# caishiqing/voice-tts

Measured on AMD Instinct MI355X. Metric: audio_seconds_per_second, higher is better.
Workload: dtype bf16

## Files before the change

### voice-tts_amd/csrc/gemm_x6.hip

```cpp
#include "common.h"

namespace ixtts {

typedef float gx_f32x16 __attribute__((ext_vector_type(16)));
typedef __bf16 gx_bf16x8 __attribute__((ext_vector_type(8)));
typedef float gx_f32x4 __attribute__((ext_vector_type(4)));
typedef unsigned int gx_u32x4 __attribute__((ext_vector_type(4)));


__global__ void gemm_x6_pack_kernel(const float* __restrict__ w, uint4* __restrict__ out, int N, int K, int Npad) {
  const long total = (long)(K / 8) * Npad;
  for (long idx = blockIdx.x * (long)blockDim.x + threadIdx.x; idx < total; idx += (long)gridDim.x * blockDim.x) {
    const int n = (int)(idx % Npad);
    const int ko = (int)(idx / Npad);
    float v[8];
#pragma unroll
    for (int e = 0; e < 8; ++e) v[e] = n < N ? w[(long)n * K + ko * 8 + e] : 0.f;
    uint4 ph, pm, pl;
    split8_bf16x3(v, ph, pm, pl);
    const int g = ko >> 1, kh = ko & 1;
    uint4* base = out + ((long)g * 6) * Npad + n;
    base[(long)(0 * 2 + kh) * Npad] = ph;
    base[(long)(1 * 2 + kh) * Npad] = pm;
    base[(long)(2 * 2 + kh) * Npad] = pl;
  }
}

__global__ __launch_bounds__(256) void gemm_x6_split_kernel(const float* __restrict__ a, long lda, uint4* __restrict__ out, int M, int K, long Mpad) {
  __shared__ float tile[64][65];
  const int r0 = blockIdx.x * 64, k0 = blockIdx.y * 64;
  const int t = threadIdx.x;
#pragma unroll
  for (int i = 0; i < 4; ++i) {
    const int r = (t >> 4) + 16 * i, kq = t & 15;
    float4 v = make_float4(0.f, 0.f, 0.f, 0.f);
    if (r0 + r < M) v = *reinterpret_cast<const float4*>(a + (long)(r0 + r) * lda + k0 + 4 * kq);
    tile[r][4 * kq + 0] = v.x; tile[r][4 * kq + 1] = v.y; tile[r][4 * kq + 2] = v.z; tile[r][4 * kq + 3] = v.w;
  }
  __syncthreads();
#pragma unroll
  for (int u = 0; u < 2; ++u) {
    const int r = t & 63, o = (t >> 6) + 4 * u;
    float v[8];
#pragma unroll
    for (int e = 0; e < 8; ++e) v[e] = tile[r][o * 8 + e];
    uint4 ph, pm, pl;
    split8_bf16x3(v, ph, pm, pl);
    const int ko = (k0 >> 3) + o, g = ko >> 1, kh = ko & 1;
    uint4* base = out + ((long)g * 6) * Mpad + r0 + r;
    base[(long)(0 * 2 + kh) * Mpad] = ph;
    base[(long)(1 * 2 + kh) * Mpad] = pm;
    base[(long)(2 * 2 + kh) * Mpad] = pl;
  }
}

enum { EPI_PLAIN = 0, EPI_SWIGLU = 1, EPI_GATE = 2 };

struct GemmX6Params {
  const uint4* Ap;
  long Mpad;
  long arow0;
  const uint4* Wp;
  const float* bias;
  float* C;
  long ldc;
  int M, N, Npad, K, accumulate, m_tiles, n_tiles;
  int tap_steps;
  int epi;
  const float* gate;
  long gate_ld, rows_per_batch;
  int nbatch;
  const int* gate_seq_off;
  unsigned long long* dbg;
};


template <int MT, int NT, int NST, int DBG = 0>
__global__ __launch_bounds__(256, (NST * (MT + NT) * 6 * 64 * 16 <= 80 * 1024) ? 2 : 1) void gemm_x6_kernel(GemmX6Params p) {
  constexpr int BM = 64 * MT, BN = 64 * NT;
  constexpr int A_UNITS = 6 * BM, W_UNITS = 6 * BN, STAGE = A_UNITS + W_UNITS;
  constexpr int NDMA = (6 * (MT + NT)) / 4;
  static_assert((6 * (MT + NT)) % 4 == 0, "the copies are dealt evenly to the 4 waves");
  constexpr int D = NST - 1;
  extern __shared__ uint4 smem[];

  const int nwg = p.m_tiles * p.n_tiles;
  const int bid = blockIdx.x;
  const int xcd = bid & 7, idx = bid >> 3;
  const int qd = nwg >> 3, rm = nwg & 7;
  const int lin = (xcd < rm ? xcd * (qd + 1) : rm * (qd + 1) + (xcd - rm) * qd) + idx;
  const int m_tile = lin / p.n_tiles, n_tile = lin - m_tile * p.n_tiles;
  const int m0 = m_tile * BM, n0 = n_tile * BN;

  const int tid = threadIdx.x, lane = tid & 63, wave = tid >> 6;
  const int wm = wave >> 1, wn = wave & 1;
  const int l31 = lane & 31, lh = lane >> 5;

  gx_f32x16 acc[MT][NT];
#pragma unroll
  for (int i = 0; i < MT; ++i)
#pragma unroll
    for (int j = 0; j < NT; ++j)
#pragma unroll
      for (int r = 0; r < 16; ++r) acc[i][j][r] = 0.f;

  const uint4* asrc = p.Ap + p.arow0 + m0 + lane;
  const uint4* wsrc = p.Wp + n0 + lane;
  auto issue = [&](int s, uint4* st) {
    const int tap = s / p.tap_steps, sa = s - tap * p.tap_steps;
#pragma unroll
    for (int q = 0; q < NDMA; ++q) {
      const int e = q * 4 + wave;
      if (e < 6 * MT) {
        const int run = e / MT, piece = e % MT;
        __builtin_amdgcn_global_load_lds((const __attribute__((address_space(1))) void*)(asrc + ((long)sa * 6 + run) * p.Mpad + tap + piece * 64),
                                         (__attribute__((address_space(3))) void*)(st + run * BM + piece * 64), 16, 0, 0);
      } else {
        const int e2 = e - 6 * MT, run = e2 / NT, piece = e2 % NT;
        __builtin_amdgcn_global_load_lds((const __attribute__((address_space(1))) void*)(wsrc + ((long)s * 6 + run) * p.Npad + piece * 64),
                                         (__attribute__((address_space(3))) void*)(st + A_UNITS + run * BN + piece * 64), 16, 0, 0);
      }
    }
  };

  const int steps = p.K >> 4;
  auto wg_stamp = [&](int k) {
    if constexpr (DBG == 3) {
      if (tid == 0) p.dbg[128 + (long)blockIdx.x * 4 + k] = __builtin_amdgcn_s_memrealtime();
    }
  };
  auto wait_younger = [&](int y) {
    if (y >= 2) asm volatile("s_waitcnt vmcnt(%0)" ::"n"(2 * NDMA) : "memory");
    else if (y == 1) asm volatile("s_waitcnt vmcnt(%0)" ::"n"(NDMA) : "memory");
    else asm volatile("s_waitcnt vmcnt(0)" ::: "memory");
  };
  static_assert(D >= 1 && D <= 3, "1..3 steps of copies in flight behind the one waited for");
  wg_stamp(0);
  for (int t = 0; t < D && t < steps; ++t) issue(t, smem + t * STAGE);
  wait_younger(min(D, steps) - 1);
  __builtin_amdgcn_s_barrier();
  asm volatile("" ::: "memory");
  wg_stamp(1);

  const unsigned base_addr = (unsigned)(uintptr_t)(const __attribute__((address_space(3))) void*)smem;
  int st_cur = 0, st_nxt = D % NST;
  for (int s = 0; s < steps; ++s) {
    auto stamp = [&](int k) {
      if constexpr (DBG == 3) {
        if (blockIdx.x == 0 && tid == 0 && s < 16) {
          p.dbg[s * 8 + k] = __builtin_amdgcn_s_memtime();
          if (k == 0) p.dbg[s * 8 + 7] = __builtin_amdgcn_s_memrealtime();
        }
      }
    };
    stamp(0);
    if (DBG != 1 && s + D < steps) issue(s + D, smem + st_nxt * STAGE);
    stamp(1);
    const unsigned cur_addr = base_addr + (unsigned)(st_cur * STAGE * 16);
    if constexpr (DBG != 2) {
      gx_u32x4 af[3][MT], bf[3][NT];
      const unsigned aaddr = cur_addr + (unsigned)((lh * BM + wm * (32 * MT) + l31) * 16);
      const unsigned waddr = cur_addr + (unsigned)((A_UNITS + lh * BN + wn * (32 * NT) + l31) * 16);
      if constexpr (MT == 4 && NT == 2) {
        asm volatile(
            "ds_read_b128 %0, %18 offset:%20\n ds_read_b128 %1, %18 offset:%21\n ds_read_b128 %2, %18 offset:%22\n ds_read_b128 %3, %18 offset:%23\n"
            "ds_read_b128 %4, %18 offset:%24\n ds_read_b128 %5, %18 offset:%25\n ds_read_b128 %6, %18 offset:%26\n ds_read_b128 %7, %18 offset:%27\n"
            "ds_read_b128 %8, %18 offset:%28\n ds_read_b128 %9, %18 offset:%29\n ds_read_b128 %10, %18 offset:%30\n ds_read_b128 %11, %18 offset:%31\n"
            "ds_read_b128 %12, %19 offset:%32\n ds_read_b128 %13, %19 offset:%33\n ds_read_b128 %14, %19 offset:%34\n ds_read_b128 %15, %19 offset:%35\n"
            "ds_read_b128 %16, %19 offset:%36\n ds_read_b128 %17, %19 offset:%37\n s_waitcnt lgkmcnt(0)"
            : "=&v"(af[0][0]), "=&v"(af[0][1]), "=&v"(af[0][2]), "=&v"(af[0][3]), "=&v"(af[1][0]), "=&v"(af[1][1]), "=&v"(af[1][2]), "=&v"(af[1][3]),
              "=&v"(af[2][0]), "=&v"(af[2][1]), "=&v"(af[2][2]), "=&v"(af[2][3]), "=&v"(bf[0][0]), "=&v"(bf[0][1]), "=&v"(bf[1][0]), "=&v"(bf[1][1]),
              "=&v"(bf[2][0]), "=&v"(bf[2][1])
            : "v"(aaddr), "v"(waddr), "n"((0 * 2 * BM + 0) * 16), "n"((0 * 2 * BM + 32) * 16), "n"((0 * 2 * BM + 64) * 16), "n"((0 * 2 * BM + 96) * 16),
              "n"((1 * 2 * BM + 0) * 16), "n"((1 * 2 * BM + 32) * 16), "n"((1 * 2 * BM + 64) * 16), "n"((1 * 2 * BM + 96) * 16), "n"((2 * 2 * BM + 0) * 16),
              "n"((2 * 2 * BM + 32) * 16), "n"((2 * 2 * BM + 64) * 16), "n"((2 * 2 * BM + 96) * 16), "n"((0 * 2 * BN + 0) * 16), "n"((0 * 2 * BN + 32) * 16),
              "n"((1 * 2 * BN + 0) * 16), "n"((1 * 2 * BN + 32) * 16), "n"((2 * 2 * BN + 0) * 16), "n"((2 * 2 * BN + 32) * 16)
            : "memory");
      } else {
        static_assert(MT == 2 && NT == 2, "fragment block written for 256 x 128 and 128 x 128 tiles");
        asm volatile(
            "ds_read_b128 %0, %12 offset:%14\n ds_read_b128 %1, %12 offset:%15\n ds_read_b128 %2, %12 offset:%16\n ds_read_b128 %3, %12 offset:%17\n"
            "ds_read_b128 %4, %12 offset:%18\n ds_read_b128 %5, %12 offset:%19\n ds_read_b128 %6, %13 offset:%20\n ds_read_b128 %7, %13 offset:%21\n"
            "ds_read_b128 %8, %13 offset:%22\n ds_read_b128 %9, %13 offset:%23\n ds_read_b128 %10, %13 offset:%24\n ds_read_b128 %11, %13 offset:%25\n"
            "s_waitcnt lgkmcnt(0)"
            : "=&v"(af[0][0]), "=&v"(af[0][1]), "=&v"(af[1][0]), "=&v"(af[1][1]), "=&v"(af[2][0]), "=&v"(af[2][1]), "=&v"(bf[0][0]), "=&v"(bf[0][1]),
              "=&v"(bf[1][0]), "=&v"(bf[1][1]), "=&v"(bf[2][0]), "=&v"(bf[2][1])
            : "v"(aaddr), "v"(waddr), "n"((0 * 2 * BM + 0) * 16), "n"((0 * 2 * BM + 32) * 16), "n"((1 * 2 * BM + 0) * 16), "n"((1 * 2 * BM + 32) * 16),
              "n"((2 * 2 * BM + 0) * 16), "n"((2 * 2 * BM + 32) * 16), "n"((0 * 2 * BN + 0) * 16), "n"((0 * 2 * BN + 32) * 16), "n"((1 * 2 * BN + 0) * 16),
              "n"((1 * 2 * BN + 32) * 16), "n"((2 * 2 * BN + 0) * 16), "n"((2 * 2 * BN + 32) * 16)
            : "memory");
      }
      stamp(2);
#pragma unroll
      for (int i = 0; i < MT; ++i)
#pragma unroll
        for (int j = 0; j < NT; ++j) {
          const gx_bf16x8 ah = __builtin_bit_cast(gx_bf16x8, af[0][i]), am = __builtin_bit_cast(gx_bf16x8, af[1][i]), al = __builtin_bit_cast(gx_bf16x8, af[2][i]);
          const gx_bf16x8 bh = __builtin_bit_cast(gx_bf16x8, bf[0][j]), bm = __builtin_bit_cast(gx_bf16x8, bf[1][j]), bl = __builtin_bit_cast(gx_bf16x8, bf[2][j]);
          acc[i][j] = __builtin_amdgcn_mfma_f32_32x32x16_bf16(al, bh, acc[i][j], 0, 0, 0);
          acc[i][j] = __builtin_amdgcn_mfma_f32_32x32x16_bf16(ah, bl, acc[i][j], 0, 0, 0);
          acc[i][j] = __builtin_amdgcn_mfma_f32_32x32x16_bf16(am, bm, acc[i][j], 0, 0, 0);
          acc[i][j] = __builtin_amdgcn_mfma_f32_32x32x16_bf16(am, bh, acc[i][j], 0, 0, 0);
          acc[i][j] = __builtin_amdgcn_mfma_f32_32x32x16_bf16(ah, bm, acc[i][j], 0, 0, 0);
          acc[i][j] = __builtin_amdgcn_mfma_f32_32x32x16_bf16(ah, bh, acc[i][j], 0, 0, 0);
        }
      if constexpr (DBG == 3) asm volatile("" ::"v"(acc[0][0][0]), "v"(acc[MT - 1][NT - 1][15]));
    }
    stamp(3);
    wait_younger(DBG == 1 ? 0 : max(0, min(D - 1, steps - s - 2)));
    stamp(4);
    __builtin_amdgcn_s_barrier();
    asm volatile("" ::: "memory");
    stamp(5);
    st_cur = st_cur + 1 == NST ? 0 : st_cur + 1;
    st_nxt = st_nxt + 1 == NST ? 0 : st_nxt + 1;
  }

  wg_stamp(2);
  if (p.epi != EPI_PLAIN) {
    static_assert(NT == 2, "pair epilogues: the wave's two 32-column blocks are the two halves");
    const int oc = (n0 + wn * 64) / 2 + l31;
    const int nh = p.N >> 1;
    if (oc < nh) {
      const float ba = p.bias != nullptr ? p.bias[n0 + wn * 64 + l31] : 0.f, bb = p.bias != nullptr ? p.bias[n0 + wn * 64 + 32 + l31] : 0.f;
#pragma unroll
      for (int i = 0; i < MT; ++i) {
        const int rbase = m0 + wm * (32 * MT) + i * 32 + 4 * lh;
#pragma unroll
        for (int r = 0; r < 16; ++r) {
          const int row = rbase + (r & 3) + 8 * (r >> 2);
          if (row < p.M) {
            float a = acc[i][0][r] + ba, b = acc[i][1][r] + bb, v;
            if (p.epi == EPI_SWIGLU) {
              v = a / (1.0f + expf(-a)) * b;
            } else {
              const long gb = p.gate_seq_off ? (long)seq_of_row(p.gate_seq_off, p.nbatch, row) : min((long)row / p.rows_per_batch, (long)p.nbatch - 1);
              const float* g = p.gate + gb * p.gate_ld;
              a += g[oc];
              b += g[nh + oc];
              v = tanhf(a) * (1.0f / (1.0f + expf(-b)));
            }
            p.C[(long)row * p.ldc + oc] = v;
          }
        }
      }
    }
  } else
#pragma unroll
  for (int j = 0; j < NT; ++j) {
    const int col = n0 + wn * (32 * NT) + j * 32 + l31;
    const bool col_ok = col < p.N;
    const float bv = (p.bias != nullptr && col_ok) ? p.bias[col] : 0.f;
#pragma unroll
    for (int i = 0; i < MT; ++i) {
      const int rbase = m0 + wm * (32 * MT) + i * 32 + 4 * lh;
#pragma unroll
      for (int r = 0; r < 16; ++r) {
        const int row = rbase + (r & 3) + 8 * (r >> 2);
        if (col_ok && row < p.M) {
          float* c = p.C + (long)row * p.ldc + col;
          float v = acc[i][j][r] + bv;
          if (p.accumulate) v += *c;
          *c = v;
        }
      }
    }
  }
  if constexpr (DBG == 3) {
    asm volatile("s_waitcnt vmcnt(0)" ::: "memory");
    wg_stamp(3);
  }
}

template <int MT, int NT, int NST, int DBG = 0>
static int launch_gemm_x6(GemmX6Params p, hipStream_t st) {
  constexpr int BM = 64 * MT, BN = 64 * NT;
  constexpr size_t smem = (size_t)NST * (6 * BM + 6 * BN) * 16;
  static_assert(smem <= 160 * 1024, "LDS stages of this tile shape");
  p.m_tiles = ceil_div(p.M, BM);
  p.n_tiles = ceil_div(p.N, BN);
  IX_ARG((long)p.n_tiles * BN <= p.Npad, "gemm_x6: packed weights padded to %d features, the %d-wide tile needs %d", p.Npad, BN, p.n_tiles * BN);
  const int taps = (p.K >> 4) / p.tap_steps;
  IX_ARG(p.arow0 + (long)p.m_tiles * BM + taps - 1 <= p.Mpad, "gemm_x6: activation planes hold %ld rows, the %d-row tiles reach row %ld", p.Mpad, BM,
         p.arow0 + (long)p.m_tiles * BM + taps - 1);
  auto kern = gemm_x6_kernel<MT, NT, NST, DBG>;
  static bool done = false;
  if (!done) {
    IX_HIP(hipFuncSetAttribute((const void*)kern, hipFuncAttributeMaxDynamicSharedMemorySize, (int)smem));
    done = true;
  }
  hipLaunchKernelGGL(kern, dim3(p.m_tiles * p.n_tiles), dim3(256), smem, st, p);
  IX_HIP(hipGetLastError());
  return IXTTS_OK;
}

}

using namespace ixtts;

extern "C" size_t ixtts_gemm_x6_packed_bytes(int N, int K) {
  if (N <= 0 || K <= 0 || K % 64) return 0;
  const size_t Npad = (size_t)(N + 255) / 256 * 256;
  return (size_t)(K / 16) * 6 * Npad * 16;
}

extern "C" int ixtts_gemm_x6_pack(const float* w_dev, void* packed_dev, int N, int K, void* stream) {
  IX_ARG(w_dev && packed_dev && N > 0 && K > 0 && K % 64 == 0, "gemm_x6_pack: bad argument (K must be a multiple of 64)");
  const int Npad = (N + 255) / 256 * 256;
  const long total = (long)(K / 8) * Npad;
  hipLaunchKernelGGL(gemm_x6_pack_kernel, dim3((unsigned)std::min<long>((total + 255) / 256, 4096)), dim3(256), 0, (hipStream_t)stream, w_dev,
                     reinterpret_cast<uint4*>(packed_dev), N, K, Npad);
  IX_HIP(hipGetLastError());
  return IXTTS_OK;
}

extern "C" long ixtts_gemm_x6_rows_padded(long rows) { return rows <= 0 ? 0 : (rows + 255) / 256 * 256 + 256; }

extern "C" int ixtts_gemm_x6_split(const float* a_dev, long lda, void* planes_dev, long rows, int K, void* stream) {
  IX_ARG(a_dev && planes_dev && rows > 0 && K > 0 && K % 64 == 0, "gemm_x6_split: bad argument (K must be a multiple of 64)");
  IX_ARG(lda >= K && lda % 4 == 0 && (reinterpret_cast<uintptr_t>(a_dev) & 15) == 0, "gemm_x6_split: rows must be 16-byte aligned (lda %ld)", lda);
  const long Mpad = ixtts_gemm_x6_rows_padded(rows);
  hipLaunchKernelGGL(gemm_x6_split_kernel, dim3((unsigned)(Mpad / 64), K / 64), dim3(256), 0, (hipStream_t)stream, a_dev, lda,
                     reinterpret_cast<uint4*>(planes_dev), (int)rows, K, Mpad);
  IX_HIP(hipGetLastError());
  return IXTTS_OK;
}

static int run_gemm_x6(GemmX6Params p, int tile, hipStream_t st) {
  if (tile == 0) {
    const long t42 = (long)ceil_div(p.M, 256) * ceil_div(p.N, 128);
    tile = t42 >= 140 ? 2 : 3;
  }
  switch (tile) {
    case 2: return launch_gemm_x6<4, 2, 2>(p, st);
    case 3: return launch_gemm_x6<2, 2, 3>(p, st);
    case 4: return launch_gemm_x6<4, 2, 4>(p, st);
    case 5: return launch_gemm_x6<2, 2, 4>(p, st);
    case 12: return launch_gemm_x6<4, 2, 2, 1>(p, st);
    case 22: return launch_gemm_x6<4, 2, 2, 2>(p, st);
    case 32: return launch_gemm_x6<4, 2, 2, 3>(p, st);
    case 33: return launch_gemm_x6<2, 2, 3, 3>(p, st);
  }
  set_error("gemm_x6: tile %d (0 auto; 2 / 3: 256x128 / 128x128, two workgroups per CU; 4 / 5: the same, one per CU with a 4-stage ring)", tile);
  return IXTTS_ERR_ARG;
}

extern "C" int ixtts_gemm_x6_f32(const void* a_planes_dev, long rows_total, long row0, const void* packed_dev, const float* bias_dev, float* c_dev,
                                 long ldc, int M, int N, int K, int accumulate, int tile, void* stream) {
  IX_ARG(a_planes_dev && packed_dev && c_dev && M > 0 && N > 0 && K > 0 && K % 64 == 0, "gemm_x6: bad argument (K must be a multiple of 64: the split pass works on 64-wide k blocks)");
  IX_ARG(ldc >= N && row0 >= 0 && row0 + M <= rows_total, "gemm_x6: rows [%ld, %ld) of %ld, ldc %ld", row0, row0 + M, rows_total, ldc);
  GemmX6Params p;
  p.Ap = reinterpret_cast<const uint4*>(a_planes_dev); p.Mpad = ixtts_gemm_x6_rows_padded(rows_total); p.arow0 = row0;
  p.Wp = reinterpret_cast<const uint4*>(packed_dev); p.bias = bias_dev; p.C = c_dev; p.ldc = ldc;
  p.M = M; p.N = N; p.Npad = (N + 255) / 256 * 256; p.K = K; p.accumulate = accumulate ? 1 : 0; p.m_tiles = p.n_tiles = 0;
  p.tap_steps = K >> 4; p.epi = EPI_PLAIN; p.gate = nullptr; p.gate_ld = 0; p.rows_per_batch = 1; p.nbatch = 1; p.gate_seq_off = nullptr;
  p.dbg = (tile == 32 || tile == 33) ? reinterpret_cast<unsigned long long*>(const_cast<float*>(bias_dev)) : nullptr;
  if (p.dbg) p.bias = nullptr;
  return run_gemm_x6(p, tile, (hipStream_t)stream);
}

extern "C" int ixtts_gemm_x6_pair_f32(const void* a_planes_dev, long rows_total, long row0, int taps, const void* packed_dev, const float* bias_dev,
                                      const float* gate_dev, long gate_ld, long rows_per_batch, int nbatch, float* c_dev, long ldc, int M, int N, int K,
                                      int epilogue, int tile, void* stream) {
  IX_ARG(a_planes_dev && packed_dev && c_dev && M > 0 && N > 0 && taps > 0 && K > 0, "gemm_x6_pair: bad argument");
  IX_ARG(K % taps == 0 && (K / taps) % 64 == 0 && N % 64 == 0, "gemm_x6_pair: K %d = %d taps of a multiple of 64, N %d a multiple of 64", K, taps, N);
  IX_ARG(epilogue == EPI_SWIGLU || (epilogue == EPI_GATE && gate_dev && rows_per_batch > 0 && nbatch > 0 && gate_ld >= N / 2),
         "gemm_x6_pair: epilogue %d (1 swiglu; 2 gate, with gate biases)", epilogue);
  IX_ARG(ldc >= N / 2 && row0 >= 0 && row0 + M + taps - 1 <= rows_total, "gemm_x6_pair: rows [%ld, %ld) + %d taps of %ld, ldc %ld", row0, row0 + M, taps,
         rows_total, ldc);
  IX_ARG(tile == 0 || tile == 2 || tile == 3, "gemm_x6_pair: tile %d (0 auto, 2, 3)", tile);
  GemmX6Params p;
  p.Ap = reinterpret_cast<const uint4*>(a_planes_dev); p.Mpad = ixtts_gemm_x6_rows_padded(rows_total); p.arow0 = row0;
  p.Wp = reinterpret_cast<const uint4*>(packed_dev); p.bias = bias_dev; p.C = c_dev; p.ldc = ldc;
  p.M = M; p.N = N; p.Npad = (N + 255) / 256 * 256; p.K = K; p.accumulate = 0; p.m_tiles = p.n_tiles = 0;
  p.tap_steps = (K / taps) >> 4; p.epi = epilogue; p.gate = gate_dev; p.gate_ld = gate_ld; p.rows_per_batch = rows_per_batch; p.nbatch = nbatch;
  p.gate_seq_off = nullptr;
  p.dbg = nullptr;
  return run_gemm_x6(p, tile, (hipStream_t)stream);
}

extern "C" int ixtts_gemm_x6_pair_gate_varlen_f32(const void* a_planes_dev, long rows_total, long row0, int taps, const void* packed_dev, const float* bias_dev,
                                                  const float* gate_dev, long gate_ld, const int* seq_off_dev, int nseq, float* c_dev, long ldc, int M, int N,
                                                  int K, int tile, void* stream) {
  IX_ARG(seq_off_dev && nseq > 0, "gemm_x6_pair_gate_varlen: null offsets table or nseq %d", nseq);
  IX_ARG(a_planes_dev && packed_dev && c_dev && gate_dev && M > 0 && N > 0 && taps > 0 && K > 0 && gate_ld >= N / 2, "gemm_x6_pair_gate_varlen: bad argument");
  IX_ARG(K % taps == 0 && (K / taps) % 64 == 0 && N % 64 == 0, "gemm_x6_pair_gate_varlen: K %d = %d taps of a multiple of 64, N %d a multiple of 64", K, taps, N);
  IX_ARG(ldc >= N / 2 && row0 >= 0 && row0 + M + taps - 1 <= rows_total, "gemm_x6_pair_gate_varlen: rows [%ld, %ld) + %d taps of %ld, ldc %ld", row0, row0 + M,
         taps, rows_total, ldc);
  IX_ARG(tile == 0 || tile == 2 || tile == 3, "gemm_x6_pair_gate_varlen: tile %d (0 auto, 2, 3)", tile);
  GemmX6Params p;
  p.Ap = reinterpret_cast<const uint4*>(a_planes_dev); p.Mpad = ixtts_gemm_x6_rows_padded(rows_total); p.arow0 = row0;
  p.Wp = reinterpret_cast<const uint4*>(packed_dev); p.bias = bias_dev; p.C = c_dev; p.ldc = ldc;
  p.M = M; p.N = N; p.Npad = (N + 255) / 256 * 256; p.K = K; p.accumulate = 0; p.m_tiles = p.n_tiles = 0;
  p.tap_steps = (K / taps) >> 4; p.epi = EPI_GATE; p.gate = gate_dev; p.gate_ld = gate_ld; p.rows_per_batch = 1; p.nbatch = nseq;
  p.gate_seq_off = seq_off_dev;
  p.dbg = nullptr;
  return run_gemm_x6(p, tile, (hipStream_t)stream);
}
```

Before: 40.91.

## Add phased 512-thread x6 GEMM kernel with split-K variant for mid-size grids

Adds a new 8-wave GEMM kernel for the bf16x3 (six-MFMA) fp32-emulation GEMM. Waves synchronise in phases around the LDS fragment reads and raise their priority during the MFMA block. A split-K variant runs two 4-wave groups on alternate K steps, each with its own stage ring, and merges their partial sums through LDS before the epilogue. Auto tile selection sends the 128x128 case with K>=2048 and 129-256 tiles to the split-K kernel, aiming to fill the CUs better where the old grid underused them. In exchange it adds extra barriers, an LDS reduction, and a new code path whose correctness must hold across all epilogues.

```diff
diff --git a/voice-tts_amd/csrc/gemm_x6.hip b/voice-tts_amd/csrc/gemm_x6.hip
--- a/voice-tts_amd/csrc/gemm_x6.hip
+++ b/voice-tts_amd/csrc/gemm_x6.hip
@@ -75,6 +75,39 @@
 };
 
 
+template <int MT, int BM, int BN>
+__device__ __forceinline__ void gx_read_frags(unsigned aaddr, unsigned waddr, gx_u32x4 (&af)[3][MT], gx_u32x4 (&bf)[3][2]) {
+  if constexpr (MT == 4) {
+    asm volatile(
+        "ds_read_b128 %0, %18 offset:%20\n ds_read_b128 %1, %18 offset:%21\n ds_read_b128 %2, %18 offset:%22\n ds_read_b128 %3, %18 offset:%23\n"
+        "ds_read_b128 %4, %18 offset:%24\n ds_read_b128 %5, %18 offset:%25\n ds_read_b128 %6, %18 offset:%26\n ds_read_b128 %7, %18 offset:%27\n"
+        "ds_read_b128 %8, %18 offset:%28\n ds_read_b128 %9, %18 offset:%29\n ds_read_b128 %10, %18 offset:%30\n ds_read_b128 %11, %18 offset:%31\n"
+        "ds_read_b128 %12, %19 offset:%32\n ds_read_b128 %13, %19 offset:%33\n ds_read_b128 %14, %19 offset:%34\n ds_read_b128 %15, %19 offset:%35\n"
+        "ds_read_b128 %16, %19 offset:%36\n ds_read_b128 %17, %19 offset:%37\n s_waitcnt lgkmcnt(0)"
+        : "=&v"(af[0][0]), "=&v"(af[0][1]), "=&v"(af[0][2]), "=&v"(af[0][3]), "=&v"(af[1][0]), "=&v"(af[1][1]), "=&v"(af[1][2]), "=&v"(af[1][3]),
+          "=&v"(af[2][0]), "=&v"(af[2][1]), "=&v"(af[2][2]), "=&v"(af[2][3]), "=&v"(bf[0][0]), "=&v"(bf[0][1]), "=&v"(bf[1][0]), "=&v"(bf[1][1]),
+          "=&v"(bf[2][0]), "=&v"(bf[2][1])
+        : "v"(aaddr), "v"(waddr), "n"((0 * 2 * BM + 0) * 16), "n"((0 * 2 * BM + 32) * 16), "n"((0 * 2 * BM + 64) * 16), "n"((0 * 2 * BM + 96) * 16),
+          "n"((1 * 2 * BM + 0) * 16), "n"((1 * 2 * BM + 32) * 16), "n"((1 * 2 * BM + 64) * 16), "n"((1 * 2 * BM + 96) * 16), "n"((2 * 2 * BM + 0) * 16),
+          "n"((2 * 2 * BM + 32) * 16), "n"((2 * 2 * BM + 64) * 16), "n"((2 * 2 * BM + 96) * 16), "n"((0 * 2 * BN + 0) * 16), "n"((0 * 2 * BN + 32) * 16),
+          "n"((1 * 2 * BN + 0) * 16), "n"((1 * 2 * BN + 32) * 16), "n"((2 * 2 * BN + 0) * 16), "n"((2 * 2 * BN + 32) * 16)
+        : "memory");
+  } else {
+    static_assert(MT == 2, "fragment block written for wave tiles of 128 x 64 and 64 x 64");
+    asm volatile(
+        "ds_read_b128 %0, %12 offset:%14\n ds_read_b128 %1, %12 offset:%15\n ds_read_b128 %2, %12 offset:%16\n ds_read_b128 %3, %12 offset:%17\n"
+        "ds_read_b128 %4, %12 offset:%18\n ds_read_b128 %5, %12 offset:%19\n ds_read_b128 %6, %13 offset:%20\n ds_read_b128 %7, %13 offset:%21\n"
+        "ds_read_b128 %8, %13 offset:%22\n ds_read_b128 %9, %13 offset:%23\n ds_read_b128 %10, %13 offset:%24\n ds_read_b128 %11, %13 offset:%25\n"
+        "s_waitcnt lgkmcnt(0)"
+        : "=&v"(af[0][0]), "=&v"(af[0][1]), "=&v"(af[1][0]), "=&v"(af[1][1]), "=&v"(af[2][0]), "=&v"(af[2][1]), "=&v"(bf[0][0]), "=&v"(bf[0][1]),
+          "=&v"(bf[1][0]), "=&v"(bf[1][1]), "=&v"(bf[2][0]), "=&v"(bf[2][1])
+        : "v"(aaddr), "v"(waddr), "n"((0 * 2 * BM + 0) * 16), "n"((0 * 2 * BM + 32) * 16), "n"((1 * 2 * BM + 0) * 16), "n"((1 * 2 * BM + 32) * 16),
+          "n"((2 * 2 * BM + 0) * 16), "n"((2 * 2 * BM + 32) * 16), "n"((0 * 2 * BN + 0) * 16), "n"((0 * 2 * BN + 32) * 16), "n"((1 * 2 * BN + 0) * 16),
+          "n"((1 * 2 * BN + 32) * 16), "n"((2 * 2 * BN + 0) * 16), "n"((2 * 2 * BN + 32) * 16)
+        : "memory");
+  }
+}
+
 template <int MT, int NT, int NST, int DBG = 0>
 __global__ __launch_bounds__(256, (NST * (MT + NT) * 6 * 64 * 16 <= 80 * 1024) ? 2 : 1) void gemm_x6_kernel(GemmX6Params p) {
   constexpr int BM = 64 * MT, BN = 64 * NT;
@@ -161,35 +194,8 @@
       gx_u32x4 af[3][MT], bf[3][NT];
       const unsigned aaddr = cur_addr + (unsigned)((lh * BM + wm * (32 * MT) + l31) * 16);
       const unsigned waddr = cur_addr + (unsigned)((A_UNITS + lh * BN + wn * (32 * NT) + l31) * 16);
-      if constexpr (MT == 4 && NT == 2) {
-        asm volatile(
-            "ds_read_b128 %0, %18 offset:%20\n ds_read_b128 %1, %18 offset:%21\n ds_read_b128 %2, %18 offset:%22\n ds_read_b128 %3, %18 offset:%23\n"
-            "ds_read_b128 %4, %18 offset:%24\n ds_read_b128 %5, %18 offset:%25\n ds_read_b128 %6, %18 offset:%26\n ds_read_b128 %7, %18 offset:%27\n"
-            "ds_read_b128 %8, %18 offset:%28\n ds_read_b128 %9, %18 offset:%29\n ds_read_b128 %10, %18 offset:%30\n ds_read_b128 %11, %18 offset:%31\n"
-            "ds_read_b128 %12, %19 offset:%32\n ds_read_b128 %13, %19 offset:%33\n ds_read_b128 %14, %19 offset:%34\n ds_read_b128 %15, %19 offset:%35\n"
-            "ds_read_b128 %16, %19 offset:%36\n ds_read_b128 %17, %19 offset:%37\n s_waitcnt lgkmcnt(0)"
-            : "=&v"(af[0][0]), "=&v"(af[0][1]), "=&v"(af[0][2]), "=&v"(af[0][3]), "=&v"(af[1][0]), "=&v"(af[1][1]), "=&v"(af[1][2]), "=&v"(af[1][3]),
-              "=&v"(af[2][0]), "=&v"(af[2][1]), "=&v"(af[2][2]), "=&v"(af[2][3]), "=&v"(bf[0][0]), "=&v"(bf[0][1]), "=&v"(bf[1][0]), "=&v"(bf[1][1]),
-              "=&v"(bf[2][0]), "=&v"(bf[2][1])
-            : "v"(aaddr), "v"(waddr), "n"((0 * 2 * BM + 0) * 16), "n"((0 * 2 * BM + 32) * 16), "n"((0 * 2 * BM + 64) * 16), "n"((0 * 2 * BM + 96) * 16),
-              "n"((1 * 2 * BM + 0) * 16), "n"((1 * 2 * BM + 32) * 16), "n"((1 * 2 * BM + 64) * 16), "n"((1 * 2 * BM + 96) * 16), "n"((2 * 2 * BM + 0) * 16),
-              "n"((2 * 2 * BM + 32) * 16), "n"((2 * 2 * BM + 64) * 16), "n"((2 * 2 * BM + 96) * 16), "n"((0 * 2 * BN + 0) * 16), "n"((0 * 2 * BN + 32) * 16),
-              "n"((1 * 2 * BN + 0) * 16), "n"((1 * 2 * BN + 32) * 16), "n"((2 * 2 * BN + 0) * 16), "n"((2 * 2 * BN + 32) * 16)
-            : "memory");
-      } else {
-        static_assert(MT == 2 && NT == 2, "fragment block written for 256 x 128 and 128 x 128 tiles");
-        asm volatile(
-            "ds_read_b128 %0, %12 offset:%14\n ds_read_b128 %1, %12 offset:%15\n ds_read_b128 %2, %12 offset:%16\n ds_read_b128 %3, %12 offset:%17\n"
-            "ds_read_b128 %4, %12 offset:%18\n ds_read_b128 %5, %12 offset:%19\n ds_read_b128 %6, %13 offset:%20\n ds_read_b128 %7, %13 offset:%21\n"
-            "ds_read_b128 %8, %13 offset:%22\n ds_read_b128 %9, %13 offset:%23\n ds_read_b128 %10, %13 offset:%24\n ds_read_b128 %11, %13 offset:%25\n"
-            "s_waitcnt lgkmcnt(0)"
-            : "=&v"(af[0][0]), "=&v"(af[0][1]), "=&v"(af[1][0]), "=&v"(af[1][1]), "=&v"(af[2][0]), "=&v"(af[2][1]), "=&v"(bf[0][0]), "=&v"(bf[0][1]),
-              "=&v"(bf[1][0]), "=&v"(bf[1][1]), "=&v"(bf[2][0]), "=&v"(bf[2][1])
-            : "v"(aaddr), "v"(waddr), "n"((0 * 2 * BM + 0) * 16), "n"((0 * 2 * BM + 32) * 16), "n"((1 * 2 * BM + 0) * 16), "n"((1 * 2 * BM + 32) * 16),
-              "n"((2 * 2 * BM + 0) * 16), "n"((2 * 2 * BM + 32) * 16), "n"((0 * 2 * BN + 0) * 16), "n"((0 * 2 * BN + 32) * 16), "n"((1 * 2 * BN + 0) * 16),
-              "n"((1 * 2 * BN + 32) * 16), "n"((2 * 2 * BN + 0) * 16), "n"((2 * 2 * BN + 32) * 16)
-            : "memory");
-      }
+      static_assert(NT == 2, "fragment block written for 256 x 128 and 128 x 128 tiles");
+      gx_read_frags<MT, BM, BN>(aaddr, waddr, af, bf);
       stamp(2);
 #pragma unroll
       for (int i = 0; i < MT; ++i)
@@ -294,6 +300,239 @@
   return IXTTS_OK;
 }
 
+template <int MT, int WM, int WN, int NST, bool KS, int DBG = 0>
+__global__ __launch_bounds__(512, 2) void gemm_x6_phased_kernel(GemmX6Params p) {
+  constexpr int BM = 32 * MT * WM, BN = 64 * WN;
+  constexpr int A_UNITS = 6 * BM, W_UNITS = 6 * BN, STAGE = A_UNITS + W_UNITS;
+  constexpr int NW = KS ? 4 : 8;
+  constexpr int PIECES = 6 * (BM + BN) / 64;
+  constexpr int NDMA = PIECES / NW;
+  constexpr int D = NST - 1;
+  static_assert(WM * WN == NW && (MT == 2 || MT == 4) && D >= 1 && D <= 2, "wave layout; at most two stages of copies behind the one waited for");
+  static_assert(!KS || MT == 2, "split K: each group finishes one of the two 32-row blocks");
+  static_assert(PIECES % NW == 0, "the copies are dealt evenly to the waves");
+  extern __shared__ uint4 smem[];
+
+  const int nwg = p.m_tiles * p.n_tiles;
+  const int bid = blockIdx.x;
+  const int xcd = bid & 7, idx = bid >> 3;
+  const int qd = nwg >> 3, rm = nwg & 7;
+  const int lin = (xcd < rm ? xcd * (qd + 1) : rm * (qd + 1) + (xcd - rm) * qd) + idx;
+  const int m_tile = lin / p.n_tiles, n_tile = lin - m_tile * p.n_tiles;
+  const int m0 = m_tile * BM, n0 = n_tile * BN;
+
+  const int tid = threadIdx.x, lane = tid & 63;
+  const int wave = __builtin_amdgcn_readfirstlane(tid >> 6);
+  const int grp = wave >> 2, wq = KS ? (wave & 3) : wave;
+  const int wm = wq / WN, wn = wq % WN;
+  const int l31 = lane & 31, lh = lane >> 5;
+
+  gx_f32x16 acc[MT][2];
+#pragma unroll
+  for (int i = 0; i < MT; ++i)
+#pragma unroll
+    for (int j = 0; j < 2; ++j)
+#pragma unroll
+      for (int r = 0; r < 16; ++r) acc[i][j][r] = 0.f;
+
+  const uint4* asrc = p.Ap + p.arow0 + m0 + lane;
+  const uint4* wsrc = p.Wp + n0 + lane;
+  auto issue = [&](int s, uint4* st) {
+    const int tap = s / p.tap_steps, sa = s - tap * p.tap_steps;
+#pragma unroll
+    for (int q = 0; q < NDMA; ++q) {
+      const int e = q * NW + wq;
+      if (e < 6 * (BM / 64)) {
+        const int run = e / (BM / 64), piece = e % (BM / 64);
+        __builtin_amdgcn_global_load_lds((const __attribute__((address_space(1))) void*)(asrc + ((long)sa * 6 + run) * p.Mpad + tap + piece * 64),
+                                         (__attribute__((address_space(3))) void*)(st + run * BM + piece * 64), 16, 0, 0);
+      } else {
+        const int e2 = e - 6 * (BM / 64), run = e2 / (BN / 64), piece = e2 % (BN / 64);
+        __builtin_amdgcn_global_load_lds((const __attribute__((address_space(1))) void*)(wsrc + ((long)s * 6 + run) * p.Npad + piece * 64),
+                                         (__attribute__((address_space(3))) void*)(st + A_UNITS + run * BN + piece * 64), 16, 0, 0);
+      }
+    }
+  };
+  auto wait_younger = [&](int y) {
+    if (y >= 2) asm volatile("s_waitcnt vmcnt(%0)" ::"n"(2 * NDMA) : "memory");
+    else if (y == 1) asm volatile("s_waitcnt vmcnt(%0)" ::"n"(NDMA) : "memory");
+    else asm volatile("s_waitcnt vmcnt(0)" ::: "memory");
+  };
+  auto slot_barrier = [&]() {
+    __builtin_amdgcn_sched_barrier(0);
+    __builtin_amdgcn_s_barrier();
+    __builtin_amdgcn_sched_barrier(0);
+  };
+  auto stamp = [&](int j, int k) {
+    if constexpr (DBG == 3) {
+      if (blockIdx.x == 0 && (tid & 255) == 0 && j < 16) p.dbg[(grp * 16 + j) * 8 + k] = __builtin_amdgcn_s_memtime();
+    }
+  };
+
+  const int nj = KS ? (p.K >> 5) : (p.K >> 4);
+  uint4* ring = smem + (KS ? grp * NST * STAGE : 0);
+  auto step_of = [&](int j) { return KS ? 2 * j + grp : j; };
+
+  for (int t = 0; t < D && t < nj; ++t) issue(step_of(t), ring + t * STAGE);
+  wait_younger(min(D, nj) - 1);
+  slot_barrier();
+  if (grp == 1) slot_barrier();
+
+  const unsigned base_addr = (unsigned)(uintptr_t)(const __attribute__((address_space(3))) void*)ring;
+  const unsigned a_off = (unsigned)((lh * BM + wm * (32 * MT) + l31) * 16), w_off = (unsigned)((A_UNITS + lh * BN + wn * 64 + l31) * 16);
+  int st_cur = 0, st_nxt = D % NST;
+  for (int j = 0; j < nj; ++j) {
+    stamp(j, 0);
+    if (j + D < nj) issue(step_of(j + D), ring + st_nxt * STAGE);
+    stamp(j, 1);
+    gx_u32x4 af[3][MT], bf[3][2];
+    const unsigned cur_addr = base_addr + (unsigned)(st_cur * STAGE * 16);
+    gx_read_frags<MT, BM, BN>(cur_addr + a_off, cur_addr + w_off, af, bf);
+    stamp(j, 2);
+    wait_younger(max(0, min(D - 1, nj - j - 2)));
+    stamp(j, 3);
+    slot_barrier();
+    stamp(j, 4);
+    __builtin_amdgcn_s_setprio(1);
+#pragma unroll
+    for (int i = 0; i < MT; ++i)
+#pragma unroll
+      for (int jj = 0; jj < 2; ++jj) {
+        const gx_bf16x8 ah = __builtin_bit_cast(gx_bf16x8, af[0][i]), am = __builtin_bit_cast(gx_bf16x8, af[1][i]), al = __builtin_bit_cast(gx_bf16x8, af[2][i]);
+        const gx_bf16x8 bh = __builtin_bit_cast(gx_bf16x8, bf[0][jj]), bm = __builtin_bit_cast(gx_bf16x8, bf[1][jj]), bl = __builtin_bit_cast(gx_bf16x8, bf[2][jj]);
+        acc[i][jj] = __builtin_amdgcn_mfma_f32_32x32x16_bf16(al, bh, acc[i][jj], 0, 0, 0);
+        acc[i][jj] = __builtin_amdgcn_mfma_f32_32x32x16_bf16(ah, bl, acc[i][jj], 0, 0, 0);
+        acc[i][jj] = __builtin_amdgcn_mfma_f32_32x32x16_bf16(am, bm, acc[i][jj], 0, 0, 0);
+        acc[i][jj] = __builtin_amdgcn_mfma_f32_32x32x16_bf16(am, bh, acc[i][jj], 0, 0, 0);
+        acc[i][jj] = __builtin_amdgcn_mfma_f32_32x32x16_bf16(ah, bm, acc[i][jj], 0, 0, 0);
+        acc[i][jj] = __builtin_amdgcn_mfma_f32_32x32x16_bf16(ah, bh, acc[i][jj], 0, 0, 0);
+      }
+    __builtin_amdgcn_s_setprio(0);
+    if constexpr (DBG == 3) asm volatile("" ::"v"(acc[0][0][0]), "v"(acc[MT - 1][1][15]));
+    stamp(j, 5);
+    if (grp == 0 || j + 1 < nj) slot_barrier();
+    stamp(j, 6);
+    st_cur = st_cur + 1 == NST ? 0 : st_cur + 1;
+    st_nxt = st_nxt + 1 == NST ? 0 : st_nxt + 1;
+  }
+
+  float* const lds_f = reinterpret_cast<float*>(smem);
+  constexpr int XCH = KS ? 2 * 4 * 2 * 16 * 64 : 0;
+  if constexpr (KS) {
+    float* mine = lds_f + ((grp * 4 + wq) * 2) * 16 * 64 + lane;
+    const float* theirs = lds_f + (((1 - grp) * 4 + wq) * 2) * 16 * 64 + lane;
+#pragma unroll
+    for (int jj = 0; jj < 2; ++jj)
+#pragma unroll
+      for (int r = 0; r < 16; ++r) mine[(jj * 16 + r) * 64] = grp == 0 ? acc[1][jj][r] : acc[0][jj][r];
+    __syncthreads();
+#pragma unroll
+    for (int jj = 0; jj < 2; ++jj)
+#pragma unroll
+      for (int r = 0; r < 16; ++r) {
+        const float o = theirs[(jj * 16 + r) * 64];
+        if (grp == 0) acc[0][jj][r] += o;
+        else acc[1][jj][r] += o;
+      }
+  }
+
+  float* const scr = lds_f + XCH + wave * (32 * 36);
+  const bool vec_ok = (reinterpret_cast<uintptr_t>(p.C) & 15) == 0 && (p.ldc & 3) == 0;
+  auto store_block = [&](const gx_f32x16& v, int row0, int col0, int ncols) {
+#pragma unroll
+    for (int r = 0; r < 16; ++r) scr[((r & 3) + 8 * (r >> 2) + 4 * lh) * 36 + l31] = v[r];
+    __builtin_amdgcn_wave_barrier();
+    const int c = col0 + 4 * (lane & 7);
+#pragma unroll
+    for (int k = 0; k < 4; ++k) {
+      const int rr = (lane >> 3) + 8 * k, row = row0 + rr;
+      float4 o = *reinterpret_cast<const float4*>(scr + rr * 36 + 4 * (lane & 7));
+      if (row < p.M) {
+        float* dst = p.C + (long)row * p.ldc + c;
+        if (vec_ok && c + 3 < ncols) {
+          if (p.accumulate) {
+            const float4 old = *reinterpret_cast<const float4*>(dst);
+            o.x += old.x; o.y += old.y; o.z += old.z; o.w += old.w;
+          }
+          *reinterpret_cast<float4*>(dst) = o;
+        } else {
+          const float e[4] = {o.x, o.y, o.z, o.w};
+#pragma unroll
+          for (int x = 0; x < 4; ++x)
+            if (c + x < ncols) dst[x] = p.accumulate ? e[x] + dst[x] : e[x];
+        }
+      }
+    }
+    __builtin_amdgcn_wave_barrier();
+  };
+  auto finish_rows = [&](const gx_f32x16& a0, const gx_f32x16& a1, int i) {
+    const int rblk = m0 + wm * (32 * MT) + i * 32;
+    if (p.epi != EPI_PLAIN) {
+      const int oc0 = (n0 + wn * 64) / 2, nh = p.N >> 1, oc = oc0 + l31;
+      const bool has_b = p.bias != nullptr && oc < nh;
+      const float ba = has_b ? p.bias[n0 + wn * 64 + l31] : 0.f, bb = has_b ? p.bias[n0 + wn * 64 + 32 + l31] : 0.f;
+      gx_f32x16 v;
+#pragma unroll
+      for (int r = 0; r < 16; ++r) {
+        const int row = rblk + 4 * lh + (r & 3) + 8 * (r >> 2);
+        float a = a0[r] + ba, b = a1[r] + bb, o = 0.f;
+        if (row < p.M && oc < nh) {
+          if (p.epi == EPI_SWIGLU) {
+            o = a / (1.0f + expf(-a)) * b;
+          } else {
+            const long gb = p.gate_seq_off ? (long)seq_of_row(p.gate_seq_off, p.nbatch, row) : min((long)row / p.rows_per_batch, (long)p.nbatch - 1);
+            const float* g = p.gate + gb * p.gate_ld;
+            a += g[oc];
+            b += g[nh + oc];
+            o = tanhf(a) * (1.0f / (1.0f + expf(-b)));
+          }
+        }
+        v[r] = o;
+      }
+      store_block(v, rblk, oc0, nh);
+    } else {
+#pragma unroll
+      for (int jj = 0; jj < 2; ++jj) {
+        const int col0 = n0 + wn * 64 + jj * 32, col = col0 + l31;
+        const float bv = (p.bias != nullptr && col < p.N) ? p.bias[col] : 0.f;
+        gx_f32x16 v;
+#pragma unroll
+        for (int r = 0; r < 16; ++r) v[r] = (jj == 0 ? a0[r] : a1[r]) + bv;
+        store_block(v, rblk, col0, p.N);
+      }
+    }
+  };
+  if constexpr (KS) {
+    if (grp == 0) finish_rows(acc[0][0], acc[0][1], 0);
+    else finish_rows(acc[1][0], acc[1][1], 1);
+  } else {
+#pragma unroll
+    for (int i = 0; i < MT; ++i) finish_rows(acc[i][0], acc[i][1], i);
+  }
+}
+
+template <int MT, int WM, int WN, int NST, bool KS, int DBG = 0>
+static int launch_gemm_x6_phased(GemmX6Params p, hipStream_t st) {
+  constexpr int BM = 32 * MT * WM, BN = 64 * WN;
+  constexpr size_t smem = (size_t)(KS ? 2 : 1) * NST * (6 * BM + 6 * BN) * 16;
+  static_assert(smem <= 160 * 1024 && smem >= (size_t)(KS ? 64 * 1024 : 0) + 8 * 32 * 36 * 4, "LDS: the stage rings, and the epilogue's areas fit into them");
+  p.m_tiles = ceil_div(p.M, BM);
+  p.n_tiles = ceil_div(p.N, BN);
+  IX_ARG((long)p.n_tiles * BN <= p.Npad, "gemm_x6: packed weights padded to %d features, the %d-wide tile needs %d", p.Npad, BN, p.n_tiles * BN);
+  const int taps = (p.K >> 4) / p.tap_steps;
+  IX_ARG(p.arow0 + (long)p.m_tiles * BM + taps - 1 <= p.Mpad, "gemm_x6: activation planes hold %ld rows, the %d-row tiles reach row %ld", p.Mpad, BM,
+         p.arow0 + (long)p.m_tiles * BM + taps - 1);
+  auto kern = gemm_x6_phased_kernel<MT, WM, WN, NST, KS, DBG>;
+  static bool done = false;
+  if (!done) {
+    IX_HIP(hipFuncSetAttribute((const void*)kern, hipFuncAttributeMaxDynamicSharedMemorySize, (int)smem));
+    done = true;
+  }
+  hipLaunchKernelGGL(kern, dim3(p.m_tiles * p.n_tiles), dim3(512), smem, st, p);
+  IX_HIP(hipGetLastError());
+  return IXTTS_OK;
+}
+
 }
 
 using namespace ixtts;
@@ -330,18 +569,24 @@
   if (tile == 0) {
     const long t42 = (long)ceil_div(p.M, 256) * ceil_div(p.N, 128);
     tile = t42 >= 140 ? 2 : 3;
+    const long t128 = (long)ceil_div(p.M, 128) * ceil_div(p.N, 128);
+    if (tile == 3 && p.K >= 2048 && t128 > 128 && t128 <= 256) tile = 8;
   }
   switch (tile) {
     case 2: return launch_gemm_x6<4, 2, 2>(p, st);
     case 3: return launch_gemm_x6<2, 2, 3>(p, st);
     case 4: return launch_gemm_x6<4, 2, 4>(p, st);
     case 5: return launch_gemm_x6<2, 2, 4>(p, st);
+    case 6: return launch_gemm_x6_phased<4, 2, 4, 3, false>(p, st);
+    case 8: return launch_gemm_x6_phased<2, 2, 2, 3, true>(p, st);
+    case 36: return launch_gemm_x6_phased<4, 2, 4, 3, false, 3>(p, st);
+    case 38: return launch_gemm_x6_phased<2, 2, 2, 3, true, 3>(p, st);
     case 12: return launch_gemm_x6<4, 2, 2, 1>(p, st);
     case 22: return launch_gemm_x6<4, 2, 2, 2>(p, st);
     case 32: return launch_gemm_x6<4, 2, 2, 3>(p, st);
     case 33: return launch_gemm_x6<2, 2, 3, 3>(p, st);
   }
-  set_error("gemm_x6: tile %d (0 auto; 2 / 3: 256x128 / 128x128, two workgroups per CU; 4 / 5: the same, one per CU with a 4-stage ring)", tile);
+  set_error("gemm_x6: tile %d (0 auto; 6 / 8: phased 256x256 / 128x128 split-K; 2 / 3: 256x128 / 128x128, two workgroups per CU; 4 / 5: the same, one per CU with a 4-stage ring)", tile);
   return IXTTS_ERR_ARG;
 }
 
@@ -354,7 +599,7 @@
   p.Wp = reinterpret_cast<const uint4*>(packed_dev); p.bias = bias_dev; p.C = c_dev; p.ldc = ldc;
   p.M = M; p.N = N; p.Npad = (N + 255) / 256 * 256; p.K = K; p.accumulate = accumulate ? 1 : 0; p.m_tiles = p.n_tiles = 0;
   p.tap_steps = K >> 4; p.epi = EPI_PLAIN; p.gate = nullptr; p.gate_ld = 0; p.rows_per_batch = 1; p.nbatch = 1; p.gate_seq_off = nullptr;
-  p.dbg = (tile == 32 || tile == 33) ? reinterpret_cast<unsigned long long*>(const_cast<float*>(bias_dev)) : nullptr;
+  p.dbg = (tile == 32 || tile == 33 || tile == 36 || tile == 38) ? reinterpret_cast<unsigned long long*>(const_cast<float*>(bias_dev)) : nullptr;
   if (p.dbg) p.bias = nullptr;
   return run_gemm_x6(p, tile, (hipStream_t)stream);
 }
@@ -368,7 +613,7 @@
          "gemm_x6_pair: epilogue %d (1 swiglu; 2 gate, with gate biases)", epilogue);
   IX_ARG(ldc >= N / 2 && row0 >= 0 && row0 + M + taps - 1 <= rows_total, "gemm_x6_pair: rows [%ld, %ld) + %d taps of %ld, ldc %ld", row0, row0 + M, taps,
          rows_total, ldc);
-  IX_ARG(tile == 0 || tile == 2 || tile == 3, "gemm_x6_pair: tile %d (0 auto, 2, 3)", tile);
+  IX_ARG(tile == 0 || tile == 2 || tile == 3 || tile == 6 || tile == 8, "gemm_x6_pair: tile %d (0 auto, 2, 3, 6, 8)", tile);
   GemmX6Params p;
   p.Ap = reinterpret_cast<const uint4*>(a_planes_dev); p.Mpad = ixtts_gemm_x6_rows_padded(rows_total); p.arow0 = row0;
   p.Wp = reinterpret_cast<const uint4*>(packed_dev); p.bias = bias_dev; p.C = c_dev; p.ldc = ldc;
@@ -387,7 +632,7 @@
   IX_ARG(K % taps == 0 && (K / taps) % 64 == 0 && N % 64 == 0, "gemm_x6_pair_gate_varlen: K %d = %d taps of a multiple of 64, N %d a multiple of 64", K, taps, N);
   IX_ARG(ldc >= N / 2 && row0 >= 0 && row0 + M + taps - 1 <= rows_total, "gemm_x6_pair_gate_varlen: rows [%ld, %ld) + %d taps of %ld, ldc %ld", row0, row0 + M,
          taps, rows_total, ldc);
-  IX_ARG(tile == 0 || tile == 2 || tile == 3, "gemm_x6_pair_gate_varlen: tile %d (0 auto, 2, 3)", tile);
+  IX_ARG(tile == 0 || tile == 2 || tile == 3 || tile == 6 || tile == 8, "gemm_x6_pair_gate_varlen: tile %d (0 auto, 2, 3, 6, 8)", tile);
   GemmX6Params p;
   p.Ap = reinterpret_cast<const uint4*>(a_planes_dev); p.Mpad = ixtts_gemm_x6_rows_padded(rows_total); p.arow0 = row0;
   p.Wp = reinterpret_cast<const uint4*>(packed_dev); p.bias = bias_dev; p.C = c_dev; p.ldc = ldc;
```

Result: faster. 41.39 (median of 6 runs) (+1.2%).
